# JiGuang283/Ray_Tracing-Rendering

Measured on AMD Instinct MI355X. Metric: Msamples/sec, Cornell Box 800x800 spp=400 MIS, higher is better.
Workload: dtype f64

## Files before the change

### ray_tracing-rendering_amd/csrc/rt_device.h

```cpp
#pragma once

#include <hip/hip_runtime.h>
#include <stdint.h>

#include "rtr_hip.h"
#include "rtr_seed.h"

#ifndef RTR_BLOCK
#define RTR_BLOCK 256
#endif

#define RT_DEV __device__ __forceinline__
#define RT_HD __host__ __device__ __forceinline__

typedef double Real;

#define RT_STATS_WORDS 82
#define RT_PROF_BASE 8
#define RT_PROF_REGIONS 37
enum { RG_OTHER = 0, RG_SETUP = 1, RG_RECTS = 2, RG_SPHERES = 3, RG_GENERIC = 4, RG_TREE = 5, RG_LEAVES = 6, RG_FINISH = 7,
       RG_SH_SETUP = 8, RG_SH_RECTS = 9, RG_SH_SPHERES = 10, RG_SH_GENERIC = 11, RG_SH_TREE = 12, RG_SH_LEAVES = 13,
       RG_MEDIA = 14, RG_MATPREP = 15, RG_SHADE_A = 16, RG_SHADE_B = 17, RG_MISS = 18, RG_REGEN = 19, RG_SHADE_RR = 20,
       RG_PARK = 21, RG_BARRIER = 22, RG_EXCHANGE = 23, RG_PAIR_SETUP = 24, RG_PAIR_RUNS = 25, RG_PAIR_SPHERES = 26,
       RG_POLL = 27, RG_BEGIN = 28, RG_SETTLE = 29, RG_COUNT = 30, RG_REJECT = 31,
// ... 1414 lines not shown
                 "v_cmpx_nlt_f64 vcc, %[a1], %[uA]\n\t"
                 "v_cmpx_ngt_f64 vcc, %[b0], %[wA]\n\t"
                 "v_cmpx_nlt_f64 vcc, %[b1], %[wA]\n\t"
                 "v_mov_b64 %[tmaxA], %[tA]\n\t"
                 "v_mov_b32 %[hitA], %[ref]\n\t"
                 "s_mov_b64 exec, %[save]\n\t"
                 "v_cmpx_ngt_f64 vcc, %[tmin], %[tB]\n\t"
                 "v_cmpx_ngt_f64 vcc, %[tB], %[tmaxB]\n\t"
                 "s_cbranch_execz .Lpx%=\n\t"
                 "v_mul_f64 %[u], %[tB], %[daB]\n\t"
                 "v_add_f64 %[u], %[oaB], %[u]\n\t"
                 "v_cmpx_ngt_f64 vcc, %[a0], %[u]\n\t"
                 "v_cmpx_nlt_f64 vcc, %[a1], %[u]\n\t"
                 "v_mul_f64 %[u], %[tB], %[dbB]\n\t"
                 "v_add_f64 %[u], %[obB], %[u]\n\t"
                 "v_cmpx_ngt_f64 vcc, %[b0], %[u]\n\t"
                 "v_cmpx_nlt_f64 vcc, %[b1], %[u]\n\t"
                 "v_mov_b64 %[tmaxB], %[tB]\n\t"
                 "v_mov_b32 %[hitB], %[ref]\n"
                 ".Lpx%=:\n\t"
                 "s_mov_b64 exec, %[save]"
                 : [u] "=&v"(u), [save] "=&s"(save), [tmaxA] "+v"(tmaxA), [hitA] "+v"(hitA), [tmaxB] "+v"(tmaxB), [hitB] "+v"(hitB)
                 : [tA] "v"(tA), [uA] "v"(uA), [wA] "v"(wA), [tB] "v"(tB), [oaB] "v"(oaB), [daB] "v"(daB), [obB] "v"(obB),
                   [dbB] "v"(dbB), [a0] "s"(a0), [a1] "s"(a1), [b0] "s"(b0), [b1] "s"(b1), [ref] "s"(ref), [tmin] "s"(tmin)
                 : "vcc");
}
struct PairRay {
    V3 o, d;
    RayDiv q;
};
template <int TYPE>
RT_DEV void pair_rects(const RT_CONST_AS double* p, int cnt, int ref, const PairRay& A, Real& tmaxA, int& hitA, const PairRay& B,
                       Real& tmaxB, int& hitB) {
    int k = 0;
    for (; k + 1 < cnt; k += 2, p += 10) {
        const Real f0 = p[0], f1 = p[1], f2 = p[2], f3 = p[3], f4 = p[4];
        const Real g0 = p[5], g1 = p[6], g2 = p[7], g3 = p[8], g4 = p[9];
        pair_rect<TYPE>(f0, f1, f2, f3, f4, ref + k, A.o, A.d, A.q, tmaxA, hitA, B.o, B.d, B.q, tmaxB, hitB);
        pair_rect<TYPE>(g0, g1, g2, g3, g4, ref + k + 1, A.o, A.d, A.q, tmaxA, hitA, B.o, B.d, B.q, tmaxB, hitB);
    }
    if (k < cnt) pair_rect<TYPE>(p[0], p[1], p[2], p[3], p[4], ref + k, A.o, A.d, A.q, tmaxA, hitA, B.o, B.d, B.q, tmaxB, hitB);
}
template <bool SPHERES = true>
RT_DEV void pair_runs(const DScene& sc, const FInst& I, const PairRay& A, Real time, Real& tmaxA, int& hitA, const PairRay& B,
                      Real& tmaxB, int& hitB) {
    const RT_CONST_AS double* p = as_const(sc.fscan) + I.scan_first;
    int ref = I.ref_first;
#pragma nounroll
    for (uint64_t runs = I.runs; runs != 0; runs >>= RT_RUN_BITS) {
        const int type = RTR_NODE_SPHERE + (int)((runs >> RT_RUN_COUNT_BITS) & 7), cnt = (int)(runs & RT_RUN_COUNT_MAX);
        RT_REGION(type >= RTR_NODE_XY_RECT ? RG_PAIR_RUNS : RG_PAIR_SPHERES);
        if (type == RTR_NODE_XY_RECT) {
            pair_rects<RTR_NODE_XY_RECT>(p, cnt, ref, A, tmaxA, hitA, B, tmaxB, hitB);
            p += 5 * cnt;
        } else if (type == RTR_NODE_XZ_RECT) {
            pair_rects<RTR_NODE_XZ_RECT>(p, cnt, ref, A, tmaxA, hitA, B, tmaxB, hitB);
            p += 5 * cnt;
        } else if (type == RTR_NODE_YZ_RECT) {
            pair_rects<RTR_NODE_YZ_RECT>(p, cnt, ref, A, tmaxA, hitA, B, tmaxB, hitB);
            p += 5 * cnt;
        } else if (type == RTR_NODE_SPHERE + RT_RUN_BOX) {
            for (int b = 0, r = ref; b < cnt; ++b, p += 6, r += 6) {
                const Real x0 = p[0], x1 = p[1], y0 = p[2], y1 = p[3], z0 = p[4], z1 = p[5];
                pair_rect<RTR_NODE_XY_RECT>(x0, x1, y0, y1, z1, r, A.o, A.d, A.q, tmaxA, hitA, B.o, B.d, B.q, tmaxB, hitB);
                pair_rect<RTR_NODE_XY_RECT>(x0, x1, y0, y1, z0, r + 1, A.o, A.d, A.q, tmaxA, hitA, B.o, B.d, B.q, tmaxB, hitB);
                pair_rect<RTR_NODE_XZ_RECT>(x0, x1, z0, z1, y1, r + 2, A.o, A.d, A.q, tmaxA, hitA, B.o, B.d, B.q, tmaxB, hitB);
                pair_rect<RTR_NODE_XZ_RECT>(x0, x1, z0, z1, y0, r + 3, A.o, A.d, A.q, tmaxA, hitA, B.o, B.d, B.q, tmaxB, hitB);
                pair_rect<RTR_NODE_YZ_RECT>(y0, y1, z0, z1, x1, r + 4, A.o, A.d, A.q, tmaxA, hitA, B.o, B.d, B.q, tmaxB, hitB);
                pair_rect<RTR_NODE_YZ_RECT>(y0, y1, z0, z1, x0, r + 5, A.o, A.d, A.q, tmaxA, hitA, B.o, B.d, B.q, tmaxB, hitB);
            }
            ref += 5 * cnt;
        } else if (SPHERES) {
            for (int k = 0; k < cnt; ++k, p += 4) {
                const V3 c = mk(p[0], p[1], p[2]);
                const Real r = p[3];
                Real t;
                if (sphere_hit_t<true>(c, r, A.o, A.d, A.q, 0.001, tmaxA, t)) tmaxA = t, hitA = ref + k;
                if (sphere_hit_t<true>(c, r, B.o, B.d, B.q, 0.001, tmaxB, t)) tmaxB = t, hitB = ref + k;
            }
        }
        ref += cnt;
    }
}
struct PairFrame {
    V3 ao, bo;
    Real adx, adz, bdx, bdz;
};
RT_HD void pair_rot(Real s, Real c, Real x, Real z, Real& rx, Real& rz) {
    rx = c * x - s * z;
    rz = s * x + c * z;
}
RT_HD PairFrame pair_frame(int shape, const double* f0, const double* f1, V3 ao, V3 ad, V3 bo, V3 bd) {
    PairFrame F;
    switch (shape) {
    case RT_SHAPE_T:
        F.ao.x = ao.x - f0[0], F.bo.x = bo.x - f0[0];
        F.ao.y = ao.y - f0[1], F.bo.y = bo.y - f0[1];
        F.ao.z = ao.z - f0[2], F.bo.z = bo.z - f0[2];
        F.adx = ad.x, F.adz = ad.z, F.bdx = bd.x, F.bdz = bd.z;
        break;
    case RT_SHAPE_R:
        pair_rot(f0[0], f0[1], ao.x, ao.z, F.ao.x, F.ao.z), pair_rot(f0[0], f0[1], bo.x, bo.z, F.bo.x, F.bo.z);
        F.ao.y = ao.y, F.bo.y = bo.y;
        pair_rot(f0[0], f0[1], ad.x, ad.z, F.adx, F.adz), pair_rot(f0[0], f0[1], bd.x, bd.z, F.bdx, F.bdz);
        break;
    case RT_SHAPE_TR: {
        const Real ax = ao.x - f0[0], bx = bo.x - f0[0];
        const Real az = ao.z - f0[2], bz = bo.z - f0[2];
        F.ao.y = ao.y - f0[1], F.bo.y = bo.y - f0[1];
        pair_rot(f1[0], f1[1], ax, az, F.ao.x, F.ao.z), pair_rot(f1[0], f1[1], bx, bz, F.bo.x, F.bo.z);
        pair_rot(f1[0], f1[1], ad.x, ad.z, F.adx, F.adz), pair_rot(f1[0], f1[1], bd.x, bd.z, F.bdx, F.bdz);
        break;
    }
    case RT_SHAPE_RT: {
        Real ax, az, bx, bz;
        pair_rot(f0[0], f0[1], ao.x, ao.z, ax, az), pair_rot(f0[0], f0[1], bo.x, bo.z, bx, bz);
        pair_rot(f0[0], f0[1], ad.x, ad.z, F.adx, F.adz), pair_rot(f0[0], f0[1], bd.x, bd.z, F.bdx, F.bdz);
        F.ao.x = ax - f1[0], F.bo.x = bx - f1[0];
        F.ao.y = ao.y - f1[1], F.bo.y = bo.y - f1[1];
        F.ao.z = az - f1[2], F.bo.z = bz - f1[2];
        break;
    }
    default:
        F.ao = ao, F.bo = bo;
        F.adx = ad.x, F.adz = ad.z, F.bdx = bd.x, F.bdz = bd.z;
        break;
    }
    return F;
}
__device__ __forceinline__ bool trace_pair_frames(const DScene& sc, V3 ao, V3 ad, Real atime, Real& a_tmax, int& a_ref, int& a_inst,
                                                  V3 bo, V3 bd, Real& b_tmax, int& b_ref, const Stack st) {
    a_ref = -1, a_inst = -1, b_ref = -1;
#ifndef RTR_NO_SHARED_DIV
    const bool ok_a = raydiv_origin_ok(ao), ok_b = raydiv_origin_ok(bo);
#else
    const bool ok_a = false, ok_b = false;
#endif
    const Real way = rcp_refined(ad.y), wby = rcp_refined(bd.y);
    const bool wa_y = rcp_safe(ad.y), wb_y = rcp_safe(bd.y);
    for (int ii = 0; ii < sc.n_finst; ++ii) {
        RT_REGION(RG_PAIR_SETUP);
        const FInst I = ld_const(sc.finst, ii);
        PairRay A, B;
        if (I.shape != RT_SHAPE_OTHER) {
            const PairFrame F = pair_frame(I.shape, I.xf_f[0], I.xf_f[1], ao, ad, bo, bd);
            A.o = F.ao, B.o = F.bo;
            A.d = mk(F.adx, ad.y, F.adz), B.d = mk(F.bdx, bd.y, F.bdz);
        } else {
            A.o = ao, A.d = ad, B.o = bo, B.d = bd;
            wrapper_enter(I.xf_type[0], I.xf_f[0], A.o, A.d);
            wrapper_enter(I.xf_type[0], I.xf_f[0], B.o, B.d);
            if (I.n_xf > 1) {
                wrapper_enter(I.xf_type[1], I.xf_f[1], A.o, A.d);
                wrapper_enter(I.xf_type[1], I.xf_f[1], B.o, B.d);
            }
            for (int k = RT_INST_XF_INLINE; k < I.n_xf; ++k) {
                const FXf x = ld_const(sc.fxf, I.xf_first + k);
                wrapper_enter(x.type, x.f, A.o, A.d);
                wrapper_enter(x.type, x.f, B.o, B.d);
            }
        }
        A.q.guard = B.q.guard = false;
        A.q.rx = rcp_refined(A.d.x), A.q.rz = rcp_refined(A.d.z);
        B.q.rx = rcp_refined(B.d.x), B.q.rz = rcp_refined(B.d.z);
        A.q.ry = way, B.q.ry = wby;
        bool sa = rcp_safe(A.d.x) & rcp_safe(A.d.z) & wa_y, sb = rcp_safe(B.d.x) & rcp_safe(B.d.z) & wb_y;
        A.q.a = A.q.ra = B.q.a = B.q.ra = 0;
        if (I.flags & RT_INST_SPHERES) {
            A.q.a = len2(A.d), B.q.a = len2(B.d);
            A.q.ra = rcp_refined(A.q.a), B.q.ra = rcp_refined(B.q.a);
            sa = sa & rcp_safe(A.q.a), sb = sb & rcp_safe(B.q.a);
        }
        if (ok_a && ok_b && __all(sa & sb)) {
            A.q.fast = B.q.fast = true;
            pair_runs(sc, I, A, atime, a_tmax, a_ref, B, b_tmax, b_ref);
        } else {
            A.q.fast = ok_a && __all(sa), B.q.fast = ok_b && __all(sb);
            int order = -1;
            if (A.q.fast)
                scan_instance<false, false, false, true>(sc, I, A.o, A.d, A.q, atime, 0.001, a_tmax, a_ref, order, st, 0);
            else
                scan_instance<false, false, false, false>(sc, I, A.o, A.d, A.q, atime, 0.001, a_tmax, a_ref, order, st, 0);
            if (B.q.fast)
                scan_instance<true, false, true, true>(sc, I, B.o, B.d, B.q, 0.0, 0.001, b_tmax, b_ref, order, st, 0);
            else
                scan_instance<true, false, true, false>(sc, I, B.o, B.d, B.q, 0.0, 0.001, b_tmax, b_ref, order, st, 0);
        }
        RT_REGION(RG_PAIR_SETUP);
        if (a_ref >= I.ref_first) a_inst = ii;
    }
    return true;
}
typedef unsigned long long PairMask;
RT_DEV PairMask pair_within(Real x, Real lo, Real hi) {
    PairMask a, b;
    asm volatile("v_cmp_ge_f64_e64 %0, |%2|, %3\n\tv_cmp_le_f64_e64 %1, |%2|, %4" : "=&s"(a), "=&s"(b) : "v"(x), "s"(lo), "s"(hi));
    return a & b;
}
RT_DEV PairMask pair_safe(Real d) { return pair_within(d, 0x1p-100, 0x1p100); }
RT_DEV PairMask pair_below(Real x, Real hi) {
    PairMask a;
    asm volatile("v_cmp_le_f64_e64 %0, |%1|, %2" : "=s"(a) : "v"(x), "s"(hi));
    return a;
}
RT_DEV PairMask pair_origin_in(V3 o) { return pair_below(o.x, 0x1p80) & pair_below(o.y, 0x1p80) & pair_below(o.z, 0x1p80); }
RT_DEV bool pair_vote(PairMask m) { return m == __builtin_amdgcn_read_exec(); }
RT_DEV bool pair_scan(const DScene& sc, const FInst& I, V3 ao, Real adx, Real ady, Real adz, Real way, V3 bo, Real bdx, Real bdy,
                      Real bdz, Real wby, PairMask sy, Real atime, Real& a_tmax, int& a_ref, Real& b_tmax, int& b_ref) {
    PairRay A, B;
    A.o = ao, B.o = bo;
    A.d = mk(adx, ady, adz), B.d = mk(bdx, bdy, bdz);
    A.q.guard = B.q.guard = false;
    A.q.fast = B.q.fast = true;
    A.q.rx = rcp_refined(adx), A.q.rz = rcp_refined(adz);
    B.q.rx = rcp_refined(bdx), B.q.rz = rcp_refined(bdz);
    A.q.ry = way, B.q.ry = wby;
    A.q.a = A.q.ra = B.q.a = B.q.ra = 0;
    const PairMask s = pair_safe(adx) & pair_safe(adz) & pair_safe(bdx) & pair_safe(bdz) & sy;
    if (I.flags & RT_INST_SPHERES) {
        Real ayy, byy;
        asm volatile("v_mul_f64 %0, %2, %2\n\tv_mul_f64 %1, %3, %3" : "=&v"(ayy), "=&v"(byy) : "v"(ady), "v"(bdy));
        A.q.a = adx * adx + ayy + adz * adz, B.q.a = bdx * bdx + byy + bdz * bdz;
        A.q.ra = rcp_refined(A.q.a), B.q.ra = rcp_refined(B.q.a);
        if (!pair_vote(s & pair_safe(A.q.a) & pair_safe(B.q.a))) return false;
        pair_runs<true>(sc, I, A, atime, a_tmax, a_ref, B, b_tmax, b_ref);
    } else {
        if (!pair_vote(s)) return false;
        pair_runs<false>(sc, I, A, atime, a_tmax, a_ref, B, b_tmax, b_ref);
    }
    return true;
}
__device__ __forceinline__ bool trace_pair_recast(const DScene& sc, V3 ao, V3 ad, Real atime, Real& a_tmax, int& a_ref, int& a_inst,
                                                  V3 bo, V3 bd, Real& b_tmax, int& b_ref) {
    a_ref = -1, a_inst = -1, b_ref = -1;
#ifdef RTR_NO_SHARED_DIV
    return false;
#endif
    if (!pair_vote(pair_origin_in(ao) & pair_origin_in(bo))) return false;
    const Real way = rcp_refined(ad.y), wby = rcp_refined(bd.y);
    const PairMask sy = pair_safe(ad.y) & pair_safe(bd.y);
    for (int ii = 0; ii < sc.n_finst; ++ii) {
        RT_REGION(RG_PAIR_SETUP);
        const FInst I = ld_const(sc.finst, ii);
        PairFrame F;
        if (I.shape != RT_SHAPE_OTHER) {
            F = pair_frame(I.shape, I.xf_f[0], I.xf_f[1], ao, ad, bo, bd);
        } else {
            V3 fad = ad, fbd = bd;
            F.ao = ao, F.bo = bo;
            wrapper_enter(I.xf_type[0], I.xf_f[0], F.ao, fad);
            wrapper_enter(I.xf_type[0], I.xf_f[0], F.bo, fbd);
            if (I.n_xf > 1) {
                wrapper_enter(I.xf_type[1], I.xf_f[1], F.ao, fad);
                wrapper_enter(I.xf_type[1], I.xf_f[1], F.bo, fbd);
            }
            for (int k = RT_INST_XF_INLINE; k < I.n_xf; ++k) {
                const FXf x = ld_const(sc.fxf, I.xf_first + k);
                wrapper_enter(x.type, x.f, F.ao, fad);
                wrapper_enter(x.type, x.f, F.bo, fbd);
            }
            F.adx = fad.x, F.adz = fad.z, F.bdx = fbd.x, F.bdz = fbd.z;
        }
        if (!pair_scan(sc, I, F.ao, F.adx, ad.y, F.adz, way, F.bo, F.bdx, bd.y, F.bdz, wby, sy, atime, a_tmax, a_ref, b_tmax, b_ref))
            return false;
        RT_REGION(RG_PAIR_SETUP);
        if (a_ref >= I.ref_first) a_inst = ii;
    }
    return true;
}
template <bool RECAST = true>
__device__ __forceinline__ bool trace_pair(const DScene& sc, V3 ao, V3 ad, Real atime, Real& a_tmax, int& a_ref, int& a_inst,
                                           V3 bo, V3 bd, Real& b_tmax, int& b_ref, const Stack st) {
#ifndef RTR_PAIR_FRAME_FALLBACK
    if (RECAST) return trace_pair_recast(sc, ao, ad, atime, a_tmax, a_ref, a_inst, bo, bd, b_tmax, b_ref);
#endif
    return trace_pair_frames(sc, ao, ad, atime, a_tmax, a_ref, a_inst, bo, bd, b_tmax, b_ref, st);
}
RT_DEV void pair_recast(const DScene& sc, V3 ao, V3 ad, Real atime, Real& a_tmax, int& a_ref, int& a_inst, V3 bo, V3 bd,
                        Real& b_tmax, int& b_ref, const Stack st) {
    RT_REGION(RG_PAIR_RECAST);
    int b_inst;
    const FSub sub = sub_scene0(sc);
    trace_fast<false, false, false, false, false>(sc, sub, ao, ad, atime, 0.001, a_tmax, a_ref, a_inst, st, 0);
    trace_fast<true, false, true, false, false>(sc, sub, bo, bd, 0.0, 0.001, b_tmax, b_ref, b_inst, st, 0);
}

template <bool UV>
__device__ __forceinline__ void fast_finish_long(const DScene& sc, V3 o, V3 d, Real time, Real t, int ref, int inst, Hit& rec) {
    const FInst I = ld_const(sc.finst, inst);
    const FRef R = ld_const(sc.fref, ref);
    V3 lo = o, ld = d;
    for (int k = 0; k < I.n_xf; ++k) {
        const FXf x = ld_const(sc.fxf, I.xf_first + k);
        wrapper_enter(x.type, x.f, lo, ld);
    }
    const rtr_node n = ld_const(sc.fprim, ref);
    const int type = n.type;
    if (type >= RTR_NODE_XY_RECT) {
        Real oa, da, ob, db;
        if (type == RTR_NODE_XY_RECT) {
            oa = lo.x, da = ld.x, ob = lo.y, db = ld.y;
        } else if (type == RTR_NODE_XZ_RECT) {
            oa = lo.x, da = ld.x, ob = lo.z, db = ld.z;
        } else {
            oa = lo.y, da = ld.y, ob = lo.z, db = ld.z;
        }
        rect_fill(n, type, lo, ld, t, oa + t * da, ob + t * db, UV, rec);
    } else {
        V3 center;
        Real radius;
        sphere_geom(n, type, time, center, radius);
        sphere_fill(n, type, center, radius, lo, ld, t, UV, rec);
    }
    int level = I.n_xf;
    for (int e = 0; e < R.n_exit; ++e) {
        const rtr_node w = ld_const(sc.nodes, as_const(sc.fexit)[R.exit_first + e]);
        V3 wd = d;
        if (w.type != RTR_NODE_FLIP_FACE) {
            V3 wo = o;
            for (int k = 0; k < level; ++k) {
                const FXf x = ld_const(sc.fxf, I.xf_first + k);
                wrapper_enter(x.type, x.f, wo, wd);
            }
            --level;
        }
        wrapper_epilogue(w, wd, rec);
    }
}
RT_DEV void xf_exit(bool rot, Real f0, Real f1, Real f2, V3 wd, Hit& rec) {
    if (!rot) {
        rec.p = add(rec.p, mk(f0, f1, f2));
        set_face_normal(rec, wd, rec.n);
    } else {
        const Real s = f0, c = f1;
        V3 p = rec.p, nn = rec.n;
        p.x = c * rec.p.x + s * rec.p.z;
        p.z = -s * rec.p.x + c * rec.p.z;
        nn.x = c * rec.n.x + s * rec.n.z;
        nn.z = -s * rec.n.x + c * rec.n.z;
        rec.p = p;
        set_face_normal(rec, wd, nn);
    }
}
RT_DEV void xf_epilogue(int type, const double* f, V3 wd, Hit& rec) {
    xf_exit(type != RTR_NODE_TRANSLATE, f[0], f[1], f[2], wd, rec);
}
template <bool UV>
RT_DEV void fast_finish_flat(const FFin* ffin, V3 o, V3 d, Real t, int ref, Hit& rec) {
    FFin F = ld_const(ffin, ref);
    asm volatile("" : "+v"(F.kind), "+v"(F.mat), "+v"(F.levels), "+v"(F.flip));
    asm volatile("" : "+v"(F.op[0][0]), "+v"(F.op[0][1]), "+v"(F.op[0][2]), "+v"(F.op[1][0]), "+v"(F.op[1][1]), "+v"(F.op[1][2]));
    asm volatile("" : "+v"(F.g[0]), "+v"(F.g[1]), "+v"(F.g[2]), "+v"(F.g[3]));
    const int n_lev = F.levels & 3;
    const bool rot0 = (F.levels & RT_FIN_ROT0) != 0, rot1 = (F.levels & RT_FIN_ROT1) != 0;
    V3 lo = o, ld = d, d1 = d;
    if (n_lev > 0) {
        xf_enter(rot0, F.op[0][0], F.op[0][1], F.op[0][2], lo, ld);
// ... 1116 lines not shown
```

### ray_tracing-rendering_amd/csrc/rt_kernels.h

```cpp
#pragma once

#include "rt_render.h"

#ifndef RTR_MEGA_WAVES
#define RTR_MEGA_WAVES 4
#endif
#ifndef RTR_PROGRAM_WAVES
#define RTR_PROGRAM_WAVES 3
#endif

constexpr int mega_waves(int integ, int trav, int ms) {
    if (ms == RT_MS_LEAN) return RTR_MEGA_WAVES;
    if (rt_is_program(trav)) return RTR_PROGRAM_WAVES;
    if (trav == RT_TRAV_MEDIA || trav == RT_TRAV_EXACT) return 2;
    if (ms == RT_MS_QUADLIT) return 3;
    if (integ == RTR_INTEGRATOR_RR || integ == RTR_INTEGRATOR_PATH) return 3;
    return 2;
}

constexpr bool pair_recasts(int ms) { return ms == RT_MS_LEAN; }

#define RT_PARK_WORDS 19
struct Park {
    double* base;
    RT_DEV V3 get3(int k) const { return mk(base[k * RTR_BLOCK], base[(k + 1) * RTR_BLOCK], base[(k + 2) * RTR_BLOCK]); }
    RT_DEV void set3(int k, V3 v) const {
        base[k * RTR_BLOCK] = v.x, base[(k + 1) * RTR_BLOCK] = v.y, base[(k + 2) * RTR_BLOCK] = v.z;
    }
    RT_DEV double get(int k) const { return base[k * RTR_BLOCK]; }
    RT_DEV void set(int k, double v) const { base[k * RTR_BLOCK] = v; }
    RT_DEV void get2(int k, uint32_t& lo, uint32_t& hi) const {
        const unsigned long long w = (unsigned long long)__double_as_longlong(base[k * RTR_BLOCK]);
        lo = (uint32_t)w, hi = (uint32_t)(w >> 32);
    }
    RT_DEV void set2(int k, uint32_t lo, uint32_t hi) const {
        base[k * RTR_BLOCK] = __longlong_as_double((long long)((unsigned long long)lo | ((unsigned long long)hi << 32)));
    }
};
enum { PK_THR = 0, PK_L = 3, PK_ACC = 6, PK_PDF = 9, PK_NCAST = 10, PK_PIXEL = 11,
       PK_CONTRIB = 12, PK_SWI = 15, PK_STMAX = 18 };
struct ParkedReq {
    bool valid;
    Park pk;
    RT_DEV void put(V3 wi, Real tmax, V3 contrib) {
        valid = true;
        pk.set3(PK_SWI, wi);
        pk.set(PK_STMAX, tmax);
        pk.set3(PK_CONTRIB, contrib);
    }
};
constexpr int park_words(int integ, int trav) {
    return (integ == RTR_INTEGRATOR_RR || integ == RTR_INTEGRATOR_PATH || rt_is_program(trav) || trav == RT_TRAV_MEDIA)
               ? 12
               : RT_PARK_WORDS;
}

constexpr bool mega_sortable(int integ, int trav, int ms) {
    return integ == RTR_INTEGRATOR_MIS && trav == RT_TRAV_FLAT && ms == RT_MS_QUADLIT;
}
constexpr bool mega_pairable(int integ, int trav) { return integ == RTR_INTEGRATOR_MIS && trav == RT_TRAV_FLAT; }
enum { SK_THR = 0, SK_L = 3, SK_PDF = 6, SK_NCLOSEST = 7, SK_NSHADOW = 8, SK_CONTRIB = 9, SK_SWI = 12, SK_STMAX = 15, SK_X = 16,
       SK_WORDS = 26 };
enum { SX_P = 0, SX_N = 3, SX_RD = 6, SX_PACK = 9 };
RT_DEV int material_class(int type) {
    return type == RTR_MAT_LAMBERTIAN ? 0 : (type == RTR_MAT_PBR ? 1 : ((type == RTR_MAT_DIELECTRIC || type == RTR_MAT_METAL) ? 2 : 3));
}

template <int ACC>
RT_DEV V3 acc_start(const RenderK& P, int slot) {
    if (!ACC) return mk(0, 0, 0);
    const double* a = P.acc_in + (size_t)slot * 3 * RTR_BLOCK + threadIdx.x;
    return mk(a[0], a[RTR_BLOCK], a[2 * RTR_BLOCK]);
}

#ifdef RTR_PHASE_CLOCKS
struct PhaseClocks {
    long long closest = 0, shade = 0, shadow = 0, other = 0, t = wall_clock64();
    RT_DEV void flush(const RenderK& P) const {
        if ((threadIdx.x & 63) == 0) {
            atomicAdd(&P.stats[3], (unsigned long long)closest);
            atomicAdd(&P.stats[4], (unsigned long long)shade);
            atomicAdd(&P.stats[5], (unsigned long long)shadow);
            atomicAdd(&P.stats[6], (unsigned long long)other);
        }
    }
};
#define RTR_CLK(phase) do { const long long now_ = wall_clock64(); clk.phase += now_ - clk.t; clk.t = now_; } while (0)
#else
struct PhaseClocks {
    RT_DEV void flush(const RenderK&) const {}
};
#define RTR_CLK(phase) do { } while (0)
#endif

#define RT_POLL_EVERY 8
RT_DEV uint32_t cancel_poll_issue(const RenderK& P, uint32_t it) {
    uint32_t word = 0;
    if ((it & (RT_POLL_EVERY - 1)) == 0) word = __hip_atomic_load(P.cancel, __ATOMIC_RELAXED, __HIP_MEMORY_SCOPE_AGENT);
    return word;
}
RT_DEV bool cancel_poll_take(const RenderK& P, uint32_t word) { return word >= P.render_id; }

template <int K_THR, int K_L, int K_PDF, int K_PIX = -1, bool JOIN = false>
// ... 180 lines not shown
                const bool go = ((back >> 32) & 1) != 0;
                ended = !go || ++ps.depth >= P.max_depth;
            }
            RT_REGION(RG_OTHER);
            if (pending) {
                pk.set(SK_NSHADOW, pk.get(SK_NSHADOW) + 1.0);
                if (!cast_shadow<TRAV>(sc, ps.ro, pk.get3(SK_SWI), pk.get(SK_STMAX), rng, st))
                    pk.set3(SK_L, add(pk.get3(SK_L), pk.get3(SK_CONTRIB)));
            }
            RT_REGION(RG_REGEN);
            if (ended) {
                const V3 L = pk.get3(SK_L);
                accp[0] += L.x, accp[RTR_BLOCK] += L.y, accp[2 * RTR_BLOCK] += L.z;
                if (ACC == 2) {
                    const double y = luminance(L);
                    q += y * y;
                }
                ++n_samples;
                ++s;
                done = s >= s_end || ((s & 7) == 0 && render_cancelled(P));
                if (!done) begin_sample<SK_THR, SK_L, SK_PDF, -1, RT_DRAW_MS(MS)>(sc, P, pk, slot, s, rng, ps);
            }
        }
        cnt.closest = (uint32_t)pk.get(SK_NCLOSEST);
        cnt.shadow = (uint32_t)pk.get(SK_NSHADOW);
    } else if (TRAV == RT_TRAV_MEDIA) {
        V3 acc = acc_start<ACC>(P, slot);
        while (!done) {
            if (fresh) {
                if ((s & 7) == 0 && render_cancelled(P)) break;
                V3 ro, rd;
                Real tm;
                camera_sample<RT_DRAW_MS(MS)>(sc, P, i, j, s, rng, ro, rd, tm);
                path_begin(ps, ro, rd, tm);
                fresh = false;
            }
            if (!bounce<INTEG, TRAV>(sc, ps, rng, st, P.max_depth, P.rr_start, cnt)) {
                acc = add(acc, ps.L);
                if (ACC == 2) {
                    const double y = luminance(ps.L);
                    q += y * y;
                }
                ++n_samples;
                ++s;
                fresh = true;
                done = s >= s_end;
            }
        }
        pk.set3(PK_ACC, acc);
    } else if (PAIR) {
        pk.set2(PK_NCAST, 0u, 0u);
        pk.set2(PK_PIXEL, (uint32_t)i, (uint32_t)j);
        pk.set3(PK_L, mk(0.0, 0.0, 0.0));
        if (!done) begin_sample<PK_THR, -1, PK_PDF, PK_PIXEL, RT_DRAW_MS(MS)>(sc, P, pk, slot, s, rng, ps);
        uint32_t it = 0;
        bool pending = false;
        bool settle = false;
        V3 so = mk(0.0, 0.0, 0.0);
        PhaseClocks clk;
        while (!done || settle) {
            RTR_CLK(other);
            RT_REGION(RG_OTHER);
            const bool cast_a = !done;
            Real a_tmax = RT_INF, b_tmax = 0.0;
            int a_ref, a_inst, b_ref;
            V3 swi = mk(1.0, 1.0, 1.0);
            RT_REGION(RG_COUNT);
            {
                uint32_t n_closest, n_shadow;
                pk.get2(PK_NCAST, n_closest, n_shadow);
                pk.set2(PK_NCAST, n_closest + (cast_a ? 1u : 0u), n_shadow + (pending ? 1u : 0u));
            }
            RT_REGION(RG_OTHER);
            if (!cast_a) {
                ps.ro = mk(0.0, 0.0, 0.0), ps.rd = mk(1.0, 1.0, 1.0), ps.tm = 0.0;
                a_tmax = 0.0;
            }
            if (pending) {
                swi = pk.get3(PK_SWI);
                b_tmax = pk.get(PK_STMAX);
            } else {
                so = mk(0.0, 0.0, 0.0);
            }
            if (!trace_pair<pair_recasts(MS)>(sc, ps.ro, ps.rd, ps.tm, a_tmax, a_ref, a_inst, so, swi, b_tmax, b_ref, st)) {
                a_tmax = cast_a ? RT_INF : 0.0;
                b_tmax = pending ? pk.get(PK_STMAX) : 0.0;
                pair_recast(sc, ps.ro, ps.rd, ps.tm, a_tmax, a_ref, a_inst, so, swi, b_tmax, b_ref, st);
            }
            RTR_CLK(closest);
            RT_REGION(RG_POLL);
            const uint32_t cancel_word = cancel_poll_issue(P, it++);
            RT_REGION(RG_SETTLE);
            const bool lit = pending && b_ref < 0;
            if (lit || settle) {
                V3 L = pk.get3(PK_L);
                if (lit) L = add(L, pk.get3(PK_CONTRIB));
                if (settle) {
                    pk.set3(PK_ACC, add(pk.get3(PK_ACC), L));
                    if (ACC == 2) {
                        const double y = luminance(L);
                        q += y * y;
                    }
                    L = mk(0.0, 0.0, 0.0);
                    settle = false;
                }
                pk.set3(PK_L, L);
            }
            pending = false;
            RTR_CLK(shadow);
            if (cast_a) {
                bool ended;
                if (a_ref < 0) {
                    RT_REGION(RG_MISS);
                    pk.set3(PK_L, add(pk.get3(PK_L), miss_radiance<INTEG, MS>(sc, pk.get3(PK_THR), ps.ro, ps.rd, ps.depth,
                                                                          ps.specular_bounce, pk.get(PK_PDF))));
                    ended = true;
                } else {
                    Hit rec;
                    rec.u = 0, rec.v = 0;
                    if (MS == RT_MS_FULL && sc.needs_uv)
                        fast_finish<true, true>(sc, ps.ro, ps.rd, ps.tm, a_tmax, a_ref, a_inst, rec);
                    else
                        fast_finish<false, true>(sc, ps.ro, ps.rd, ps.tm, a_tmax, a_ref, a_inst, rec);
                    ps.thr = pk.get3(PK_THR);
                    ps.L = mk(0.0, 0.0, 0.0);
                    ps.prev_bsdf_pdf = pk.get(PK_PDF);
                    const V3 wo = neg(unit(ps.rd));
                    ParkedReq rq{false, pk};
                    const MatCtx mc = mat_prepare<MS>(sc, rec);
                    shade_a_mis<MS, INTEG>(sc, ps, rec, mc, wo, rng, rq);
                    pending = rq.valid;
                    const bool go = shade_b_mis<MS, INTEG>(sc, ps, rec, mc, wo, rng, P.rr_start);
                    RT_REGION(RG_PARK);
                    ps.ro = rec.p;
                    so = rec.p;
                    pk.set3(PK_THR, ps.thr);
                    if (ps.L.x != 0.0 || ps.L.y != 0.0 || ps.L.z != 0.0) pk.set3(PK_L, add(pk.get3(PK_L), ps.L));
                    pk.set(PK_PDF, ps.prev_bsdf_pdf);
                    ended = !go || ++ps.depth >= P.max_depth;
                }
                RTR_CLK(shade);
                RT_REGION(RG_REGEN);
                if (ended) {
                    settle = true;
                    ++n_samples;
                    ++s;
                    done = s >= s_end;
                    RT_REGION(RG_BEGIN);
                    if (!done) begin_sample<PK_THR, -1, PK_PDF, PK_PIXEL, RT_DRAW_MS(MS)>(sc, P, pk, slot, s, rng, ps);
                }
            }
            RT_REGION(RG_POLL);
            if (cancel_poll_take(P, cancel_word)) done = true;
        }
        pk.get2(PK_NCAST, cnt.closest, cnt.shadow);
        clk.flush(P);
    } else {
        pk.set2(PK_NCAST, 0u, 0u);
        pk.set2(PK_PIXEL, (uint32_t)i, (uint32_t)j);
        if (!done) begin_sample<PK_THR, PK_L, PK_PDF, PK_PIXEL, RT_DRAW_MS(MS)>(sc, P, pk, slot, s, rng, ps);
        PhaseClocks clk;
        uint32_t it = 0;
        while (!done) {
            bool pending = false, ended = false;
            bool shadowed = false;
            RTR_CLK(other);
            RT_REGION(RG_OTHER);
// ... 210 lines not shown
        qw.samples += (unsigned long long)__builtin_popcountll(__ballot(now)) * (unsigned long long)(qb.s1 - qb.s0);
        const int taken = qw.next + (int)__builtin_popcountll(m);
        qw.next = taken < RT_QUEUE_JOBS ? taken : RT_QUEUE_JOBS;
        m = __ballot(need);
    }
    slot.set(qw);
    return got;
}

RT_DEV void pair_retire(const Park& pk, V3& so) {
    pk.set3(PK_SWI, mk(1.0, 1.0, 1.0));
    so = mk(0.0, 0.0, 0.0);
}

template <int INTEG, int TRAV, int MS>
__global__ void __launch_bounds__(RTR_BLOCK, mega_waves(INTEG, TRAV, MS))
    k_mega_queue(const DScene* __restrict__ scp, const RenderK P, const int stack_words, uint32_t* __restrict__ ,
                 const int ) {
    static_assert(mega_pairable(INTEG, TRAV), "no pair-cast variant of this kernel");
    extern __shared__ int lds_stack[];
    const DScene& sc = *scp;
    const Stack st{lds_stack + threadIdx.x};
    const Park pk{reinterpret_cast<double*>(lds_stack + stack_words * RTR_BLOCK) + threadIdx.x};
    int* const my_cell = lds_stack + threadIdx.x;
    const QueueSlot slot;
#ifdef RTR_REGION_PROFILE
    if (threadIdx.x < 4 * 2 * RT_PROF_REGIONS + 8) rt_prof_lds[threadIdx.x] = 0;
    if (threadIdx.x + 256 < 4 * 2 * RT_PROF_REGIONS + 8) rt_prof_lds[threadIdx.x + 256] = 0;
    __syncthreads();
    if ((threadIdx.x & 63) == 0) rt_prof_lds[4 * 2 * RT_PROF_REGIONS + (threadIdx.x >> 6) * 2] = __builtin_readcyclecounter();
#endif
    PathCounters cnt;
    cnt.closest = 0, cnt.shadow = 0;
    PathState ps;
    uint32_t rng = 1;
    int s = 0;
    slot.set(QueueWave{0, RT_QUEUE_JOBS, 0ull});
    pk.set3(PK_ACC, mk(0.0, 0.0, 0.0));
    pk.set2(PK_NCAST, 0u, 0u);
    pk.set3(PK_L, mk(0.0, 0.0, 0.0));
    pk.set3(PK_SWI, mk(1.0, 1.0, 1.0));
    pk.set(PK_STMAX, 0.0);
    *my_cell = -1;
    QueueCamera::set(camera_div_make(P.W, P.H));
    bool done;
    {
        const QueueArgs Q = queue_args();
        done = !queue_take(Q.P, Q.q_counter, Q.n_blocks, slot, true, pk, my_cell, s);
    }
    if (!done) {
        uint32_t lo, hi;
        int i, j, s_end;
        pk.get2(PK_PIXEL, lo, hi);
        queue_unpack(lo, hi, i, j, s_end);
        camera_sample<RT_DRAW_MS(MS)>(sc, QueueCamera::get(P.W, P.H), P.seed, P.W, i, j, s, rng, ps.ro, ps.rd, ps.tm);
        ps.depth = 0, ps.specular_bounce = false;
        pk.set3(PK_THR, mk(1.0, 1.0, 1.0));
        pk.set(PK_PDF, 0.0);
    }
    uint32_t it = 0;
    bool pending = false;
    bool settle = false;
    V3 so = mk(0.0, 0.0, 0.0);
    PhaseClocks clk;
    while (!done || settle) {
        RTR_CLK(other);
        RT_REGION(RG_OTHER);
        const bool cast_a = !done;
        Real a_tmax = RT_INF;
        int a_ref, a_inst, b_ref;
        RT_REGION(RG_COUNT);
        {
            uint32_t n_closest, n_shadow;
            pk.get2(PK_NCAST, n_closest, n_shadow);
            pk.set2(PK_NCAST, n_closest + (cast_a ? 1u : 0u), n_shadow + (pending ? 1u : 0u));
        }
        RT_REGION(RG_OTHER);
        if (!cast_a) {
            ps.ro = mk(0.0, 0.0, 0.0), ps.rd = mk(1.0, 1.0, 1.0), ps.tm = 0.0;
            a_tmax = 0.0;
        }
        const V3 swi = pk.get3(PK_SWI);
        Real b_tmax = pk.get(PK_STMAX);
        if (!trace_pair<pair_recasts(MS)>(sc, ps.ro, ps.rd, ps.tm, a_tmax, a_ref, a_inst, so, swi, b_tmax, b_ref, st)) {
            a_tmax = cast_a ? RT_INF : 0.0;
            b_tmax = pk.get(PK_STMAX);
            pair_recast(sc, ps.ro, ps.rd, ps.tm, a_tmax, a_ref, a_inst, so, swi, b_tmax, b_ref, st);
            pair_retire(pk, so);
        }
        RTR_CLK(closest);
        RT_REGION(RG_POLL);
        const uint32_t cancel_word = cancel_poll_issue(P, it++);
        RT_REGION(RG_SETTLE);
        const bool lit = pending && b_ref < 0;
        if (lit || settle) {
            V3 L = pk.get3(PK_L);
            if (lit) L = add(L, pk.get3(PK_CONTRIB));
            if (settle) {
                pk.set3(PK_ACC, add(pk.get3(PK_ACC), L));
                L = mk(0.0, 0.0, 0.0);
                settle = false;
            }
            pk.set3(PK_L, L);
        }
        pending = false;
        {
            Real dead = 0.0;
            asm volatile("" : "+v"(dead));
            pk.set(PK_STMAX, dead);
        }
        RTR_CLK(shadow);
        bool begin = false;
        if (cast_a) {
            bool ended;
            if (a_ref < 0) {
                RT_REGION(RG_MISS);
                pk.set3(PK_L, add(pk.get3(PK_L), miss_radiance<INTEG, MS>(sc, pk.get3(PK_THR), ps.ro, ps.rd, ps.depth,
                                                                      ps.specular_bounce, pk.get(PK_PDF))));
                ended = true;
            } else {
                Hit rec;
                rec.u = 0, rec.v = 0;
                if (MS == RT_MS_FULL && sc.needs_uv)
                    fast_finish<true, true>(sc, ps.ro, ps.rd, ps.tm, a_tmax, a_ref, a_inst, rec);
                else
                    fast_finish<false, true>(sc, ps.ro, ps.rd, ps.tm, a_tmax, a_ref, a_inst, rec);
                ps.thr = pk.get3(PK_THR);
                ps.L = mk(0.0, 0.0, 0.0);
                ps.prev_bsdf_pdf = pk.get(PK_PDF);
                const V3 wo = neg(unit(ps.rd));
                ParkedReq rq{false, pk};
                const MatCtx mc = mat_prepare<MS>(sc, rec);
                shade_a_mis<MS, INTEG>(sc, ps, rec, mc, wo, rng, rq);
                pending = rq.valid;
                const bool go = shade_b_mis<MS, INTEG>(sc, ps, rec, mc, wo, rng, P.rr_start);
                RT_REGION(RG_PARK);
                ps.ro = rec.p;
                so = rec.p;
                pk.set3(PK_THR, ps.thr);
                if (ps.L.x != 0.0 || ps.L.y != 0.0 || ps.L.z != 0.0) pk.set3(PK_L, add(pk.get3(PK_L), ps.L));
                pk.set(PK_PDF, ps.prev_bsdf_pdf);
                ended = !go || ++ps.depth >= P.max_depth;
            }
            RTR_CLK(shade);
            RT_REGION(RG_REGEN);
            if (ended) {
                settle = true;
                ++s;
                begin = true;
            }
        }
        const bool job_end = !cast_a && *my_cell >= 0;
        if (__ballot(job_end)) {
            RT_REGION(RG_EXCHANGE);
            const QueueArgs Q = queue_args();
            if (job_end) {
                uint32_t lo, hi;
                pk.get2(PK_PIXEL, lo, hi);
                const V3 acc = pk.get3(PK_ACC);
                const int cell = *my_cell;
                double* out = Q.P.partial + (size_t)cell * 3 * RTR_BLOCK + ((lo >> 12) & 0xf0u) + (lo & 0xfu);
                out[0] = acc.x;
                out[RTR_BLOCK] = acc.y;
                out[2 * RTR_BLOCK] = acc.z;
                atomicAdd(&Q.P.done[cell], 1);
                pk.set3(PK_ACC, mk(0.0, 0.0, 0.0));
            }
// ... 487 lines not shown
```

Before: 6207.

## Add hand-written inline-asm pair run scanner for rect/box runs in lean mode

Adds pair_runs_lean, an inline-assembly loop that decodes the run words on scalar registers, loads rect and box parameters with scalar loads, and intersects two rays against axis-aligned rects using exec-masked compares and early branch-out for the second ray. The lean multi-sample path uses it in place of the templated C++ pair_runs for scenes without spheres. The aim is to cut instruction count, branching and register pressure in the hottest rect-intersection loop. It hardcodes SGPR ranges and the run encoding, which may clash with compiler register allocation and is harder to maintain.

```diff
diff --git a/ray_tracing-rendering_amd/csrc/rt_device.h b/ray_tracing-rendering_amd/csrc/rt_device.h
--- a/ray_tracing-rendering_amd/csrc/rt_device.h
+++ b/ray_tracing-rendering_amd/csrc/rt_device.h
@@ -1520,6 +1520,138 @@
         ref += cnt;
     }
 }
+#define RT_PL_SIDE(N, W1, A0, A1, B0, B1, K, OK, DK, RK, OA, DA, OB, DB)                                                       \
+    "v_add_f64 %[nA], " K ", -%[a" OK "]\n\t"                                                                                   \
+    "v_add_f64 %[nB], " K ", -%[b" OK "]\n\t"                                                                                   \
+    "v_mul_f64 %[tA], %[nA], %[a" RK "]\n\t"                                                                                    \
+    "v_mul_f64 %[tB], %[nB], %[b" RK "]\n\t"                                                                                    \
+    "v_fma_f64 %[nA], -%[a" DK "], %[tA], %[nA]\n\t"                                                                            \
+    "v_fma_f64 %[nB], -%[b" DK "], %[tB], %[nB]\n\t"                                                                            \
+    "v_fma_f64 %[tA], %[nA], %[a" RK "], %[tA]\n\t"                                                                             \
+    "v_fma_f64 %[tB], %[nB], %[b" RK "], %[tB]\n\t"                                                                             \
+    "v_mul_f64 %[uA], %[tA], %[a" DA "]\n\t"                                                                                    \
+    "v_mul_f64 %[wA], %[tA], %[a" DB "]\n\t"                                                                                    \
+    "v_add_f64 %[uA], %[a" OA "], %[uA]\n\t"                                                                                    \
+    "v_add_f64 %[wA], %[a" OB "], %[wA]\n\t" W1 "\n\t"                                                                          \
+    "v_cmpx_ngt_f64 vcc, %[tmin], %[tA]\n\t"                                                                                    \
+    "v_cmpx_ngt_f64 vcc, %[tA], %[tmaxA]\n\t"                                                                                   \
+    "v_cmpx_ngt_f64 vcc, " A0 ", %[uA]\n\t"                                                                                     \
+    "v_cmpx_nlt_f64 vcc, " A1 ", %[uA]\n\t"                                                                                     \
+    "v_cmpx_ngt_f64 vcc, " B0 ", %[wA]\n\t"                                                                                     \
+    "v_cmpx_nlt_f64 vcc, " B1 ", %[wA]\n\t"                                                                                     \
+    "v_mov_b64 %[tmaxA], %[tA]\n\t"                                                                                             \
+    "v_mov_b32 %[hitA], %[ref]\n\t"                                                                                             \
+    "s_mov_b64 exec, %[save]\n\t"                                                                                               \
+    "v_cmpx_ngt_f64 vcc, %[tmin], %[tB]\n\t"                                                                                    \
+    "v_cmpx_ngt_f64 vcc, %[tB], %[tmaxB]\n\t"                                                                                   \
+    "s_cbranch_execz .Lplx%=_" #N "\n\t"                                                                                        \
+    "v_mul_f64 %[u], %[tB], %[b" DA "]\n\t"                                                                                     \
+    "v_add_f64 %[u], %[b" OA "], %[u]\n\t"                                                                                      \
+    "v_cmpx_ngt_f64 vcc, " A0 ", %[u]\n\t"                                                                                      \
+    "v_cmpx_nlt_f64 vcc, " A1 ", %[u]\n\t"                                                                                      \
+    "v_mul_f64 %[u], %[tB], %[b" DB "]\n\t"                                                                                     \
+    "v_add_f64 %[u], %[b" OB "], %[u]\n\t"                                                                                      \
+    "v_cmpx_ngt_f64 vcc, " B0 ", %[u]\n\t"                                                                                      \
+    "v_cmpx_nlt_f64 vcc, " B1 ", %[u]\n\t"                                                                                      \
+    "v_mov_b64 %[tmaxB], %[tB]\n\t"                                                                                             \
+    "v_mov_b32 %[hitB], %[ref]\n"                                                                                               \
+    ".Lplx%=_" #N ":\n\t"                                                                                                       \
+    "s_mov_b64 exec, %[save]\n\t"                                                                                               \
+    "s_add_u32 %[ref], %[ref], 1\n\t"
+#define RT_PL_XY(N, W1, A0, A1, B0, B1, K) RT_PL_SIDE(N, W1, A0, A1, B0, B1, K, "oz", "dz", "rz", "ox", "dx", "oy", "dy")
+#define RT_PL_XZ(N, W1, A0, A1, B0, B1, K) RT_PL_SIDE(N, W1, A0, A1, B0, B1, K, "oy", "dy", "ry", "ox", "dx", "oz", "dz")
+#define RT_PL_YZ(N, W1, A0, A1, B0, B1, K) RT_PL_SIDE(N, W1, A0, A1, B0, B1, K, "ox", "dx", "rx", "oy", "dy", "oz", "dz")
+#define RT_PL_RECTS(T, L, N0, N1, N2)                                                                                           \
+    ".Lpl" L "%=:\n\t"                                                                                                          \
+    "s_cmp_lt_u32 %[cnt], 2\n\t"                                                                                                \
+    "s_cbranch_scc1 .Lpl" L "1%=\n"                                                                                             \
+    ".Lpl" L "2%=:\n\t"                                                                                                         \
+    "s_load_dwordx16 s[16:31], %[p], %[off]\n\t"                                                                                \
+    "s_load_dwordx4 s[32:35], %[p], %[off] offset:64\n\t"                                                                       \
+    "s_waitcnt lgkmcnt(0)\n\t"                                                                                                  \
+    T(N0, "s_sub_u32 %[cnt], %[cnt], 2", "s[16:17]", "s[18:19]", "s[20:21]", "s[22:23]", "s[24:25]")                           \
+    T(N1, "s_add_u32 %[off], %[off], 80", "s[26:27]", "s[28:29]", "s[30:31]", "s[32:33]", "s[34:35]")                          \
+    "s_cmp_gt_u32 %[cnt], 1\n\t"                                                                                                \
+    "s_cbranch_scc1 .Lpl" L "2%=\n"                                                                                             \
+    ".Lpl" L "1%=:\n\t"                                                                                                         \
+    "s_cmp_eq_u32 %[cnt], 0\n\t"                                                                                                \
+    "s_cbranch_scc1 .Lplrun%=\n\t"                                                                                              \
+    "s_load_dwordx8 s[16:23], %[p], %[off]\n\t"                                                                                 \
+    "s_load_dwordx2 s[24:25], %[p], %[off] offset:32\n\t"                                                                       \
+    "s_waitcnt lgkmcnt(0)\n\t"                                                                                                  \
+    T(N2, "s_add_u32 %[off], %[off], 40", "s[16:17]", "s[18:19]", "s[20:21]", "s[22:23]", "s[24:25]")                          \
+    "s_branch .Lplrun%=\n"
+typedef unsigned PairRegs16 __attribute__((ext_vector_type(16)));
+typedef unsigned PairRegs4 __attribute__((ext_vector_type(4)));
+RT_DEV void pair_runs_lean(const DScene& sc, const FInst& I, const PairRay& A, Real& tmaxA, int& hitA, const PairRay& B, Real& tmaxB,
+                           int& hitB) {
+    const RT_CONST_AS double* p = as_const(sc.fscan) + I.scan_first;
+    const Real tmin = 0.001;
+    unsigned lo = (unsigned)I.runs, hi = (unsigned)(I.runs >> 32);
+    int ref = I.ref_first;
+    Real nA, nB, tA, tB, uA, wA, u;
+    unsigned long long save;
+    unsigned off, cnt, typ;
+    PairRegs16 r16;
+    PairRegs4 r4;
+    static_assert(RT_RUN_BITS == 8 && RT_RUN_COUNT_BITS == 5 && RT_RUN_COUNT_MAX == 31 && RT_RUN_BOX == 5 &&
+                      RTR_NODE_XY_RECT - RTR_NODE_SPHERE == 2 && RTR_NODE_XZ_RECT - RTR_NODE_SPHERE == 3 &&
+                      RTR_NODE_YZ_RECT - RTR_NODE_SPHERE == 4,
+                  "pair_runs_lean decodes the run word with these numbers");
+    RT_REGION(RG_PAIR_RUNS);
+    asm volatile("s_mov_b64 %[save], exec\n\t"
+                 "s_mov_b32 %[off], 0\n"
+                 ".Lplrun%=:\n\t"
+                 "s_cmp_lg_u32 %[lo], 0\n\t"
+                 "s_cbranch_scc1 .Lpldec%=\n\t"
+                 "s_mov_b32 %[lo], %[hi]\n\t"
+                 "s_mov_b32 %[hi], 0\n\t"
+                 "s_cmp_eq_u32 %[lo], 0\n\t"
+                 "s_cbranch_scc1 .Lplend%=\n"
+                 ".Lpldec%=:\n\t"
+                 "s_and_b32 %[cnt], %[lo], 31\n\t"
+                 "s_bfe_u32 %[typ], %[lo], 0x30005\n\t"
+                 "s_lshr_b32 %[lo], %[lo], 8\n\t"
+                 "s_cmp_eq_u32 %[typ], 5\n\t"
+                 "s_cbranch_scc1 .Lplbox%=\n\t"
+                 "s_cmp_eq_u32 %[typ], 4\n\t"
+                 "s_cbranch_scc1 .Lplyz%=\n\t"
+                 "s_cmp_eq_u32 %[typ], 3\n\t"
+                 "s_cbranch_scc1 .Lplxz%=\n\t"
+                 "s_cmp_eq_u32 %[typ], 2\n\t"
+                 "s_cbranch_scc0 .Lplend%=\n"
+                 RT_PL_RECTS(RT_PL_XY, "xy", 0, 1, 2)
+                 RT_PL_RECTS(RT_PL_XZ, "xz", 3, 4, 5)
+                 RT_PL_RECTS(RT_PL_YZ, "yz", 6, 7, 8)
+                 ".Lplbox%=:\n\t"
+                 "s_load_dwordx8 s[16:23], %[p], %[off]\n\t"
+                 "s_load_dwordx4 s[24:27], %[p], %[off] offset:32\n\t"
+                 "s_waitcnt lgkmcnt(0)\n\t"
+                 RT_PL_XY(9, "s_add_u32 %[off], %[off], 48", "s[16:17]", "s[18:19]", "s[20:21]", "s[22:23]", "s[26:27]")
+                 RT_PL_XY(10, "s_sub_u32 %[cnt], %[cnt], 1", "s[16:17]", "s[18:19]", "s[20:21]", "s[22:23]", "s[24:25]")
+                 RT_PL_XZ(11, "s_nop 0", "s[16:17]", "s[18:19]", "s[24:25]", "s[26:27]", "s[22:23]")
+                 RT_PL_XZ(12, "s_nop 0", "s[16:17]", "s[18:19]", "s[24:25]", "s[26:27]", "s[20:21]")
+                 RT_PL_YZ(13, "s_nop 0", "s[20:21]", "s[22:23]", "s[24:25]", "s[26:27]", "s[18:19]")
+                 RT_PL_YZ(14, "s_nop 0", "s[20:21]", "s[22:23]", "s[24:25]", "s[26:27]", "s[16:17]")
+                 "s_cmp_lg_u32 %[cnt], 0\n\t"
+                 "s_cbranch_scc1 .Lplbox%=\n\t"
+                 "s_branch .Lplrun%=\n"
+                 ".Lplend%=:"
+                 : [tmaxA] "+v"(tmaxA), [hitA] "+v"(hitA), [tmaxB] "+v"(tmaxB), [hitB] "+v"(hitB), [lo] "+s"(lo), [hi] "+s"(hi),
+                   [ref] "+s"(ref), [nA] "=&v"(nA), [nB] "=&v"(nB), [tA] "=&v"(tA), [tB] "=&v"(tB), [uA] "=&v"(uA), [wA] "=&v"(wA),
+                   [u] "=&v"(u), [save] "=&s"(save), [off] "=&s"(off), [cnt] "=&s"(cnt), [typ] "=&s"(typ), "=&{s[16:31]}"(r16),
+                   "=&{s[32:35]}"(r4)
+                 : [aox] "v"(A.o.x), [aoy] "v"(A.o.y), [aoz] "v"(A.o.z), [adx] "v"(A.d.x), [ady] "v"(A.d.y), [adz] "v"(A.d.z),
+                   [arx] "v"(A.q.rx), [ary] "v"(A.q.ry), [arz] "v"(A.q.rz), [box] "v"(B.o.x), [boy] "v"(B.o.y), [boz] "v"(B.o.z),
+                   [bdx] "v"(B.d.x), [bdy] "v"(B.d.y), [bdz] "v"(B.d.z), [brx] "v"(B.q.rx), [bry] "v"(B.q.ry), [brz] "v"(B.q.rz),
+                   [p] "s"(p), [tmin] "s"(tmin)
+                 : "vcc", "scc");
+}
+#undef RT_PL_RECTS
+#undef RT_PL_XY
+#undef RT_PL_XZ
+#undef RT_PL_YZ
+#undef RT_PL_SIDE
 struct PairFrame {
     V3 ao, bo;
     Real adx, adz, bdx, bdz;
@@ -1643,6 +1775,7 @@
 }
 RT_DEV PairMask pair_origin_in(V3 o) { return pair_below(o.x, 0x1p80) & pair_below(o.y, 0x1p80) & pair_below(o.z, 0x1p80); }
 RT_DEV bool pair_vote(PairMask m) { return m == __builtin_amdgcn_read_exec(); }
+template <bool ROUTINE>
 RT_DEV bool pair_scan(const DScene& sc, const FInst& I, V3 ao, Real adx, Real ady, Real adz, Real way, V3 bo, Real bdx, Real bdy,
                       Real bdz, Real wby, PairMask sy, Real atime, Real& a_tmax, int& a_ref, Real& b_tmax, int& b_ref) {
     PairRay A, B;
@@ -1664,10 +1797,14 @@
         pair_runs<true>(sc, I, A, atime, a_tmax, a_ref, B, b_tmax, b_ref);
     } else {
         if (!pair_vote(s)) return false;
-        pair_runs<false>(sc, I, A, atime, a_tmax, a_ref, B, b_tmax, b_ref);
+        if (ROUTINE)
+            pair_runs_lean(sc, I, A, a_tmax, a_ref, B, b_tmax, b_ref);
+        else
+            pair_runs<false>(sc, I, A, atime, a_tmax, a_ref, B, b_tmax, b_ref);
     }
     return true;
 }
+template <bool ROUTINE>
 __device__ __forceinline__ bool trace_pair_recast(const DScene& sc, V3 ao, V3 ad, Real atime, Real& a_tmax, int& a_ref, int& a_inst,
                                                   V3 bo, V3 bd, Real& b_tmax, int& b_ref) {
     a_ref = -1, a_inst = -1, b_ref = -1;
@@ -1699,18 +1836,22 @@
             }
             F.adx = fad.x, F.adz = fad.z, F.bdx = fbd.x, F.bdz = fbd.z;
         }
-        if (!pair_scan(sc, I, F.ao, F.adx, ad.y, F.adz, way, F.bo, F.bdx, bd.y, F.bdz, wby, sy, atime, a_tmax, a_ref, b_tmax, b_ref))
+        if (!pair_scan<ROUTINE>(sc, I, F.ao, F.adx, ad.y, F.adz, way, F.bo, F.bdx, bd.y, F.bdz, wby, sy, atime, a_tmax, a_ref, b_tmax, b_ref))
             return false;
         RT_REGION(RG_PAIR_SETUP);
         if (a_ref >= I.ref_first) a_inst = ii;
     }
     return true;
 }
-template <bool RECAST = true>
+template <bool RECAST = true, bool ROUTINE = RECAST>
 __device__ __forceinline__ bool trace_pair(const DScene& sc, V3 ao, V3 ad, Real atime, Real& a_tmax, int& a_ref, int& a_inst,
                                            V3 bo, V3 bd, Real& b_tmax, int& b_ref, const Stack st) {
 #ifndef RTR_PAIR_FRAME_FALLBACK
-    if (RECAST) return trace_pair_recast(sc, ao, ad, atime, a_tmax, a_ref, a_inst, bo, bd, b_tmax, b_ref);
+#ifdef RTR_PAIR_RUNS_PLAIN
+    if (RECAST) return trace_pair_recast<false>(sc, ao, ad, atime, a_tmax, a_ref, a_inst, bo, bd, b_tmax, b_ref);
+#else
+    if (RECAST) return trace_pair_recast<ROUTINE>(sc, ao, ad, atime, a_tmax, a_ref, a_inst, bo, bd, b_tmax, b_ref);
+#endif
 #endif
     return trace_pair_frames(sc, ao, ad, atime, a_tmax, a_ref, a_inst, bo, bd, b_tmax, b_ref, st);
 }
diff --git a/ray_tracing-rendering_amd/csrc/rt_kernels.h b/ray_tracing-rendering_amd/csrc/rt_kernels.h
--- a/ray_tracing-rendering_amd/csrc/rt_kernels.h
+++ b/ray_tracing-rendering_amd/csrc/rt_kernels.h
@@ -19,6 +19,7 @@
 }
 
 constexpr bool pair_recasts(int ms) { return ms == RT_MS_LEAN; }
+constexpr bool pair_runs_routine(int ms) { return ms == RT_MS_LEAN; }
 
 #define RT_PARK_WORDS 19
 struct Park {
@@ -365,7 +366,7 @@
             } else {
                 so = mk(0.0, 0.0, 0.0);
             }
-            if (!trace_pair<pair_recasts(MS)>(sc, ps.ro, ps.rd, ps.tm, a_tmax, a_ref, a_inst, so, swi, b_tmax, b_ref, st)) {
+            if (!trace_pair<pair_recasts(MS), pair_runs_routine(MS)>(sc, ps.ro, ps.rd, ps.tm, a_tmax, a_ref, a_inst, so, swi, b_tmax, b_ref, st)) {
                 a_tmax = cast_a ? RT_INF : 0.0;
                 b_tmax = pending ? pk.get(PK_STMAX) : 0.0;
                 pair_recast(sc, ps.ro, ps.rd, ps.tm, a_tmax, a_ref, a_inst, so, swi, b_tmax, b_ref, st);
@@ -742,7 +743,7 @@
         }
         const V3 swi = pk.get3(PK_SWI);
         Real b_tmax = pk.get(PK_STMAX);
-        if (!trace_pair<pair_recasts(MS)>(sc, ps.ro, ps.rd, ps.tm, a_tmax, a_ref, a_inst, so, swi, b_tmax, b_ref, st)) {
+        if (!trace_pair<pair_recasts(MS), pair_runs_routine(MS)>(sc, ps.ro, ps.rd, ps.tm, a_tmax, a_ref, a_inst, so, swi, b_tmax, b_ref, st)) {
             a_tmax = cast_a ? RT_INF : 0.0;
             b_tmax = pk.get(PK_STMAX);
             pair_recast(sc, ps.ro, ps.rd, ps.tm, a_tmax, a_ref, a_inst, so, swi, b_tmax, b_ref, st);
```

Result: faster. 6421 (median of 6 runs) (+3.4%).
